# v-manhlt3/Disentangle-VAE-for-VC

Measured on AMD Instinct MI355X. Metric: utterances/sec (B=64, 80-mel, T=128) train step, higher is better.
Workload: dtype f32; 1 GPU; configs[1]: train step, B=64 pairs/GPU, 80-mel, T=128, 10 synthetic speakers, speaker_size=4, latent=32, Adam lr=1e-4; fp32 tensors, master weights, BatchNorm, losses and Adam; compute_mode=fp32x3, global_batch=64, frames=128, parallelism=dp1, launch=hipGraph replay, params=94930304

## Files before the change

disentangle-vae-for-vc_amd/_lib.py:

```python
from __future__ import annotations

import ctypes as C
import os
import subprocess

import torch

_HERE = os.path.dirname(os.path.abspath(__file__))
LIB_PATH = os.environ.get("DVAE_LIB_PATH") or os.path.join(_HERE, "libdvae_hip.so")
_lib = None

vp, i32, i64, f32 = C.c_void_p, C.c_int, C.c_int64, C.c_float


class Ranges(C.Structure):
    _fields_ = [("lo", i64 * 8), ("hi", i64 * 8), ("n", i32)]


class LstmDir(C.Structure):
    _fields_ = [("gates", vp), ("w_hh", vp), ("h_out", vp), ("c_all", vp), ("dh_out", vp),
                ("dgates", vp), ("dc_ws", vp), ("w_packed", vp), ("reverse", i32), ("packed_mode", i32),
                ("step_shift", i32), ("state_bf16", i32), ("pers_ws", vp), ("pers_timeout_us", C.c_uint), ("dbias_ih", vp), ("dbias_hh", vp), ("dbias_part", vp), ("gate_ld", i64)]


# ... 49 lines not shown
    "dvae_bn_ws_bytes": (i64, [i32, i32, i32]),
    "dvae_bn_stats_fwd": (i32, [vp, vp, vp, vp, vp, vp, vp, i32, i32, i32, i32, f32, f32, vp]),
    "dvae_bn_apply_fwd": (i32, [vp, vp, vp, vp, vp, vp, vp, i32, i32, i32, i32, i32, i32, vp]),
    "dvae_bn_bwd": (i32, [vp, vp, vp, vp, vp, vp, vp, vp, vp, vp, i32, i32, i32, i32, i32, i32, vp]),
    "dvae_bn_bwd_from_y": (i32, [vp, vp, vp, vp, vp, vp, vp, vp, vp, vp, i32, i32, i32, i32, i32, i32, vp]),
    "dvae_lstm_pack_w": (i32, [vp, vp, vp, i32, vp]),
    "dvae_lstm_pack_w_bf16": (i32, [vp, vp, vp, i32, vp]),
    "dvae_lstm_pack_w_x3": (i32, [vp, vp, vp, i32, vp]),
    "dvae_repack_all": (i32, [C.POINTER(RepackDesc), i32, vp]),
    "dvae_lstm_pers_supported": (i32, [i32, i32, i32, i32]),
    "dvae_lstm_pers_ws_bytes": (i64, [i32, i32]),
    "dvae_lstm_pers_check": (i32, [vp, C.POINTER(i32), vp]),
    "dvae_lstm_pers_selftest": (i32, [C.POINTER(LstmDir), i32, i32, i32, i64, i32, vp]),
    "dvae_lstm_seq_fwd": (i32, [C.POINTER(LstmDir), i32, i32, i32, i32, i64, vp]),
    "dvae_lstm_seq_bwd": (i32, [C.POINTER(LstmDir), i32, i32, i32, i32, i64, vp]),
    "dvae_lstm_seq_fwd_range": (i32, [C.POINTER(LstmDir), i32, i32, i32, i32, i64, i32, i32, vp]),
    "dvae_lstm_seq_bwd_range": (i32, [C.POINTER(LstmDir), i32, i32, i32, i32, i64, i32, i32, vp]),
    "dvae_latent_fwd": (i32, [vp] * 9 + [i32, i32, i32, vp]),
    "dvae_latent_bwd": (i32, [vp] * 11 + [i32, i32, i32, vp]),
    "dvae_kl_fwd": (i32, [vp, vp, vp, i64, f32, vp]),
    "dvae_kl_bwd": (i32, [vp, vp, vp, vp, vp, i64, f32, vp]),
    "dvae_l1_ws_bytes": (i64, [i64]),
    "dvae_l1_sum_fwd": (i32, [vp, vp, vp, vp, i64, f32, vp]),
    "dvae_l1_sum_bwd": (i32, [vp, vp, vp, vp, i64, f32, vp]),
    "dvae_loss_ws_bytes": (i64, [i64]),
    "dvae_loss_fwd": (i32, [C.POINTER(LossDesc), vp, vp, vp]),
    "dvae_loss_bwd": (i32, [C.POINTER(LossDesc), vp] + [vp] * 10 + [vp]),
    "dvae_loss_fwd_sched": (i32, [C.POINTER(LossDesc), C.POINTER(LossSched), vp, vp, vp, vp]),
    "dvae_loss_bwd_sched": (i32, [C.POINTER(LossDesc), C.POINTER(LossSched), vp, vp] + [vp] * 10 + [vp]),
    "dvae_gemm_f32_batched": (i32, [vp, vp, vp, i32, i32, i32, i32, i64, i64, i64, i32, i32, i32, i32, i32, vp]),
    "dvae_gemm_f32_slabs": (i32, [vp, vp, vp, vp, i64, i32, vp, i32, i32, i32, i64, i64, i64, i32, i32, i32, i32, i32, vp]),
    "dvae_gemm_f32_batched_slabs": (i32, [vp, vp, vp, i32, vp, i64, i32, i32, i32, i32, i64, i64, i64, i32, i32, i32, i32,
                                          i32, vp]),
    "dvae_conv5_fwd_slabs": (i32, [vp, vp, vp, vp, vp, i64, i32, i32, i32, i32, i32, i32, vp]),
    "dvae_conv5_dgrad_t_slabs": (i32, [vp, vp, vp, vp, i64, i32, i32, i32, i32, i32, i32, vp]),
    "dvae_conv5_wgrad_slabs": (i32, [vp, vp, vp, vp, i64, i32, i32, i32, i32, i32, i32, i32, i32, vp]),
    "dvae_slab_sum": (i32, [vp, vp, i64, i32, i64, i32, i32, vp]),
    "dvae_slab_fold": (i32, [C.POINTER(SlabDesc), i32, vp]),
    "dvae_colsum_ws_bytes": (i64, [i32, i32]),
    "dvae_colsum_add_ws": (i32, [vp, vp, vp, i32, i32, i64, i32, vp, vp]),
    "dvae_adam_flat": (i32, [vp, vp, vp, vp, i64, f32, f32, f32, f32, f32, i32, vp]),
    "dvae_adam_flat_dev": (i32, [vp, vp, vp, vp, i64, f32, f32, f32, vp, vp, vp, i32, vp]),
    "dvae_adam_flat_dev_clip": (i32, [vp, vp, vp, vp, i64, f32, f32, f32, vp, vp, vp, i32, vp, vp]),
    "dvae_grad_sumsq_ws_bytes": (i64, [i64]),
    "dvae_grad_sumsq": (i32, [vp, i64, vp, vp]),
    "dvae_grad_clip_finalize": (i32, [vp, i64, vp, vp, vp, i32, vp]),
    "dvae_ema_tick": (i32, [vp, vp, vp, vp]),
    "dvae_ema_update": (i32, [vp, vp, i64, vp, vp]),
    "dvae_swap_f32": (i32, [vp, vp, i64, vp]),
    "dvae_lstm_pers_err_word": (vp, [vp]),
    "dvae_sum_f32": (i32, [vp, vp, vp, vp, i64, vp]),
    "dvae_zero_f32": (i32, [vp, i64, vp]),
    "dvae_mel_to_frames": (i32, [vp, vp, vp, i32, i32, i32, i32, vp]),
    "dvae_frames_to_mel": (i32, [vp, vp, i32, i32, i32, vp]),
    "dvae_permute_102": (i32, [vp, vp, i32, i32, i32, vp]),
    "dvae_colsum_add": (i32, [vp, vp, vp, i32, i32, i64, i32, vp]),
    "dvae_transpose": (i32, [vp, vp, i32, i32, vp]),
    "dvae_act_fwd": (i32, [vp, i64, i32, vp]),
    "dvae_act_bwd": (i32, [vp, vp, vp, i64, i32, vp]),
    "dvae_gather_crop": (i32, [vp, vp, vp, vp, vp, i32, i32, i32, i32, vp]),
    "dvae_mel_to_chunks": (i32, [vp, vp, i32, i32, i32, i32, vp]),
    "dvae_chunks_to_mel": (i32, [vp, vp, i32, i32, i32, f32, f32, i32, vp]),
    "dvae_conversion_latents": (i32, [vp, vp, vp, vp, vp, i32, i32, i32, i32, vp]),
    "dvae_mul_div": (i32, [vp, vp, vp, vp, i64, vp]),
    "dvae_mel_to_windows": (i32, [vp, i64, vp, vp, vp, i32, i32, i32, vp]),
    "dvae_window_latents": (i32, [vp, vp, vp, vp, vp, C.c_double, vp, i32, i32, i32, i32, vp]),
# ... 124 lines not shown
```

disentangle-vae-for-vc_amd/csrc/gemm.hip:

```cpp
#include <cstdlib>
#include <type_traits>
#include <utility>
#include "common.h"
#include "gemm_common.h"

#ifndef DVAE_X3_PD
#define DVAE_X3_PD 2
#endif

int g_dvae_compute_mode = 0;
int g_dvae_deterministic = 0;

#if defined(DVAE_GEMM_TS) || defined(DVAE_GEMM_TS2)
__device__ unsigned long long g_gemm_ts[1024 * 8];
#define TS_NOW() __builtin_amdgcn_s_memtime()
#endif

__device__ __attribute__((aligned(16))) float g_gemm_zero[4] = {0.f, 0.f, 0.f, 0.f};

namespace {

template <bool A_KC, bool B_KC, int NTW, int BK, int WG, int MODE = 0, bool BNS = false, bool A16 = false, bool B16M = false>
__global__ __launch_bounds__(64 * WG * WG) void gemm_f32_kernel(const GemmParams p) {
  constexpr bool BF = (MODE == 1), X3 = (MODE == 2);
// ... 448 lines not shown
          const int dr = (r & 3) + 8 * (r >> 2);
          if (row0 + dr < p.M) cbase[(int64_t)dr * p.ldc] += acc[mt][nt][r] + bias_v;
        }
      } else {
#pragma unroll
        for (int r = 0; r < 16; ++r) {
          const int dr = (r & 3) + 8 * (r >> 2);
          if (row0 + dr < p.M) atomicAdd(cbase + (int64_t)dr * p.ldc, acc[mt][nt][r] + bias_v);
        }
      }
    }
  }
  if constexpr (BNS) {
    const int chunk = tile_m * 2 + wm, nchunks = (p.M + DVAE_BN_ROWS_PER_CHUNK - 1) / DVAE_BN_ROWS_PER_CHUNK;
#pragma unroll
    for (int nt = 0; nt < NTW; ++nt) {
      const int col = n0 + wn * 32 * NTW + nt * 32 + l31;
#pragma unroll
      for (int q = 0; q < 4; ++q) bst[nt][q] += __shfl_xor(bst[nt][q], 32, 64);
      if (kh == 0 && col < p.N && chunk < nchunks) {
        double* o = p.bn_part + ((int64_t)chunk * p.bn_groups * p.N + col) * 2;
        o[0] = (double)bst[nt][0];
        o[1] = (double)bst[nt][1];
        if (p.bn_groups > 1) {
          o[(int64_t)p.N * 2] = (double)bst[nt][2];
          o[(int64_t)p.N * 2 + 1] = (double)bst[nt][3];
        }
      }
    }
  }
}


template <bool A_KC, bool B_KC, bool BNS, bool BNU = false>
__global__ __launch_bounds__(256) void gemm_x3_tall_kernel(const GemmParams p) {
  constexpr int BM = 256, BN = 128, BK = 16, NTHR = 256, MTW = 4, NTW = 2;
  constexpr int LD_KC = BK + 8;
  constexpr int LDA = A_KC ? LD_KC : BM + 32;
  constexpr int LDB = B_KC ? LD_KC : BN + 32;
  constexpr int A_SZ = A_KC ? BM * LD_KC : BK * LDA;
  constexpr int B_SZ = B_KC ? BN * LD_KC : BK * LDB;
  constexpr int NUA = BM * BK / 8 / NTHR, NUB = BN * BK / 8 / NTHR;
  constexpr int NU = NUA + NUB;
  constexpr unsigned OOB = 0xC0000000u;
  __shared__ __attribute__((aligned(16))) __bf16 As[2][3 * A_SZ];
  __shared__ __attribute__((aligned(16))) __bf16 Bs[2][3 * B_SZ];
  typedef unsigned u32x4 __attribute__((ext_vector_type(4)));

  const int t = threadIdx.x;
  const int lane = t & 63, wave = t >> 6;
  const int wm = wave >> 1, wn = wave & 1;
  const int l31 = lane & 31, kh = lane >> 5;
#ifdef DVAE_GEMM_TS2
  const unsigned long long t2_entry = __builtin_amdgcn_s_memrealtime();
#endif

  int tile_m, tile_n;
  gemm_tile_of(p, tile_m, tile_n);
  const int m0 = tile_m * BM, n0 = tile_n * BN;
  int tap_fixed = 0, ks = blockIdx.z;
  if (p.tap_mode == 2) {
    tap_fixed = blockIdx.z % p.taps;
    ks = blockIdx.z / p.taps;
  }
  const int k_begin = ks * p.k_per_split;
  const int k_end = min(p.K, k_begin + p.k_per_split);
  const int kiters = (k_end - k_begin) / BK;
  const int n_iters = (p.tap_mode == 1 ? p.taps : 1) * kiters;
  const bool to_slab = p.slab != nullptr && p.split_k > 1;
  float* __restrict__ C = (to_slab ? p.slab + (int64_t)ks * p.slab_stride : (float*)p.C) +
                          (p.tap_mode == 2 ? (int64_t)tap_fixed * p.c_tap_stride : 0);

  const int a_rows = A_KC ? p.M : p.K, b_rows = B_KC ? p.N : p.K;
  const __amdgpu_buffer_rsrc_t a_rs = __builtin_amdgcn_make_buffer_rsrc((void*)p.A, 0, (int)((int64_t)a_rows * p.lda * 4), 0x00020000);
  const int64_t b_bytes = (int64_t)b_rows * p.ldb * 4 * ((p.tap_mode == 1) ? p.taps : 1);
  const __amdgpu_buffer_rsrc_t b_rs = __builtin_amdgcn_make_buffer_rsrc((void*)p.B, 0, (int)b_bytes, 0x00020000);
  unsigned a_vo[NUA], b_vo[NUB];
  int a_off[NUA], b_off[NUB];
#pragma unroll
  for (int j = 0; j < NUA; ++j) {
    const int idx = t + NTHR * j;
    if (A_KC) {
      const int row = idx >> 1, k8 = (idx & 1) * 8;
      a_off[j] = row * LDA + k8;
      a_vo[j] = (unsigned)(((int64_t)(m0 + row) * p.lda + k_begin + k8) * 4);
      if (m0 + row >= p.M) a_vo[j] = OOB;
    } else {
      const int kr = idx / (BM / 8), m8 = (idx % (BM / 8)) * 8;
      a_off[j] = kr * LDA + m8;
      a_vo[j] = (unsigned)(((int64_t)(k_begin + kr) * p.lda + m0 + m8) * 4);
      if (m0 + m8 >= p.M) a_vo[j] = OOB;
    }
  }
  const int64_t b_shift = (p.tap_mode == 2) ? (int64_t)(tap_fixed - 2) * p.bk_row_shift : 0;
#pragma unroll
  for (int j = 0; j < NUB; ++j) {
    const int idx = t + NTHR * j;
    if (B_KC) {
      const int row = idx >> 1, k8 = (idx & 1) * 8;
      b_off[j] = row * LDB + k8;
      b_vo[j] = (unsigned)(((int64_t)(n0 + row) * p.ldb + k_begin + k8) * 4);
      if (n0 + row >= p.N) b_vo[j] = OOB;
    } else {
      const int kr = idx / (BN / 8), n8 = (idx % (BN / 8)) * 8;
      b_off[j] = kr * LDB + n8;
      b_vo[j] = (unsigned)(((int64_t)(k_begin + kr) + b_shift) * p.ldb * 4 + (int64_t)(n0 + n8) * 4);
      if (n0 + n8 >= p.N) b_vo[j] = OOB;
    }
  }
  const int ntaps_loop = (p.tap_mode == 1) ? p.taps : 1;
  const int a_tap_step = (p.tap_mode == 1) ? (int)(p.a_row_shift * p.lda * 4) : 0;
  const int b_tap_step = (p.tap_mode == 1) ? (int)(p.b_tap_stride * 4) : 0;
  const int a_k_step = A_KC ? BK * 4 : (int)(BK * p.lda * 4);
  const int b_k_step = B_KC ? BK * 4 : (int)(BK * p.ldb * 4);
  int tap_n = 0, kit_n = 0;
  struct Regs {
    u32x4 a[NUA][2], b[NUB][2];
  };
  auto load_tiles = [&](Regs& g) {
    const bool live = kit_n < kiters;
    const unsigned a_s = live ? (unsigned)((tap_n - 2) * a_tap_step + kit_n * a_k_step) : OOB;
    const unsigned b_s = live ? (unsigned)(tap_n * b_tap_step + kit_n * b_k_step) : OOB;
#pragma unroll
    for (int j = 0; j < NUA; ++j) {
      g.a[j][0] = __builtin_amdgcn_raw_buffer_load_b128(a_rs, a_vo[j] + a_s, 0, 0);
      g.a[j][1] = __builtin_amdgcn_raw_buffer_load_b128(a_rs, a_vo[j] + a_s, 16, 0);
    }
// ... 47 lines not shown
  f32x16 acc[MTW][NTW];
#pragma unroll
  for (int i = 0; i < MTW; ++i)
#pragma unroll
    for (int j = 0; j < NTW; ++j)
#pragma unroll
      for (int r = 0; r < 16; ++r) acc[i][j][r] = 0.f;

  Regs gs[2];
  Frags fr[2];
  load_tiles(gs[0]);
  load_tiles(gs[1]);
  stage_all(0, gs[0]);
  load_tiles(gs[0]);
  __syncthreads();
  read_frags(fr[0], 0);
  stage_all(1, gs[1]);
  __syncthreads();

  constexpr int ia[6] = {0, 0, 1, 1, 0, 2}, ib[6] = {0, 1, 0, 1, 2, 0};
  unsigned a_s = 0, b_s = 0;
  unsigned pl[2][3][4];
  float rr[2][8];
  auto unit_regs = [&](Regs& g, int j) -> const u32x4(&)[2] { return j < NUA ? g.a[j] : g.b[j - NUA]; };
  auto fsub = [](float a, float b) {
    float r;
    asm("v_sub_f32 %0, %1, %2" : "=v"(r) : "v"(a), "v"(b));
    return r;
  };
  auto step = [&](auto G, auto U) {
    constexpr int g = decltype(G)::value, u = decltype(U)::value;
    {
      constexpr int term = g / 8, mt = (g % 8) / 2, nt = g % 2;
      acc[mt][nt] = __builtin_amdgcn_mfma_f32_32x32x16_bf16(fr[u].a[mt][ia[term]], fr[u].b[nt][ib[term]], acc[mt][nt], 0, 0, 0);
    }
    if constexpr (g < 6) {
      Regs& gn = gs[u ^ 1];
      constexpr int j = g / 2, hv = g % 2;
      if constexpr (j < NUA) gn.a[j][hv] = __builtin_amdgcn_raw_buffer_load_b128(a_rs, a_vo[j] + a_s, 16 * hv, 0);
      else gn.b[j - NUA][hv] = __builtin_amdgcn_raw_buffer_load_b128(b_rs, b_vo[j - NUA] + b_s, 16 * hv, 0);
    }
    if constexpr (g < 18) {
      Frags& f = fr[u ^ 1];
      constexpr int q = g / 6, w = g % 6;
      if constexpr (w < MTW) f.a[w][q] = frag(&As[u ^ 1][q * A_SZ], A_KC, LDA, wm * 128 + w * 32);
      else f.b[w - MTW][q] = frag(&Bs[u ^ 1][q * B_SZ], B_KC, LDB, wn * 64 + (w - MTW) * 32);
    } else {
      constexpr int s = g - 18;
      constexpr int SPU = 9;
      constexpr int j = s / SPU, w = s % SPU;
      if constexpr (j < NU) {
        const u32x4(&v)[2] = unit_regs(gs[u], j);
        if constexpr (w < 8) {
          constexpr int lvl = w / 4, i = w % 4;
          if constexpr (lvl == 0) {
            const f32x4 xv = __builtin_bit_cast(f32x4, v[i / 2]);
            rr[j & 1][2 * i] = xv[2 * (i % 2)];
            rr[j & 1][2 * i + 1] = xv[2 * (i % 2) + 1];
          }
          const f32x2 xy = {rr[j & 1][2 * i], rr[j & 1][2 * i + 1]};
          const unsigned pk = __builtin_bit_cast(unsigned, __builtin_convertvector(xy, bf16x2));
          pl[j & 1][lvl][i] = pk;
          rr[j & 1][2 * i] = fsub(rr[j & 1][2 * i], __builtin_bit_cast(float, pk << 16));
          rr[j & 1][2 * i + 1] = fsub(rr[j & 1][2 * i + 1], __builtin_bit_cast(float, pk & 0xffff0000u));
        } else {
#pragma unroll
          for (int i = 0; i < 4; ++i) {
// ... 151 lines not shown
            }
          }
        }
      }
      if constexpr (BNS) {
        const int chunk = tile_m * 4 + wm * 2 + half, nchunks = (p.M + DVAE_BN_ROWS_PER_CHUNK - 1) / DVAE_BN_ROWS_PER_CHUNK;
        bool second = false;
        if constexpr (BNU) second = ((m0 + wm * 128 + half * 64) % p.bn_nseg) >= p.bn_nseg / p.bn_groups;
#pragma unroll
        for (int nt = 0; nt < NTW; ++nt) {
          if (second) {
            bst[nt][2] = bst[nt][0];
            bst[nt][3] = bst[nt][1];
            bst[nt][0] = bst[nt][1] = 0.f;
          }
          const int col = n0 + wn * 64 + nt * 32 + l31;
#pragma unroll
          for (int q = 0; q < 4; ++q) bst[nt][q] += __shfl_xor(bst[nt][q], 32, 64);
          if (kh == 0 && col < p.N && chunk < nchunks) {
            double* o = p.bn_part + ((int64_t)chunk * p.bn_groups * p.N + col) * 2;
            o[0] = (double)bst[nt][0];
            o[1] = (double)bst[nt][1];
            if (p.bn_groups > 1) {
              o[(int64_t)p.N * 2] = (double)bst[nt][2];
              o[(int64_t)p.N * 2 + 1] = (double)bst[nt][3];
            }
          }
        }
      }
    }
  };
  using std::integral_constant;
  const int epi_here = to_slab ? DVAE_EPI_STORE : p.epi;
  if (epi_here == DVAE_EPI_ATOMIC) emit(integral_constant<int, DVAE_EPI_ATOMIC>{}, integral_constant<int, DVAE_ACT_NONE>{});
  else if (epi_here == DVAE_EPI_ACCUM) emit(integral_constant<int, DVAE_EPI_ACCUM>{}, integral_constant<int, DVAE_ACT_NONE>{});
  else if (p.act == DVAE_ACT_NONE) emit(integral_constant<int, DVAE_EPI_STORE>{}, integral_constant<int, DVAE_ACT_NONE>{});
  else if (p.act == DVAE_ACT_RELU) emit(integral_constant<int, DVAE_EPI_STORE>{}, integral_constant<int, DVAE_ACT_RELU>{});
  else emit(integral_constant<int, DVAE_EPI_STORE>{}, integral_constant<int, DVAE_ACT_TANH>{});
#ifdef DVAE_GEMM_TS2
  asm volatile("s_waitcnt vmcnt(0)" ::: "memory");
  const unsigned flat_wg = blockIdx.z * gridDim.x + blockIdx.x;
  if ((threadIdx.x & 63) == 0 && flat_wg < 256) {
    unsigned long long* o = g_gemm_ts + (flat_wg * 4 + wave) * 8;
    o[0] = t2_entry; o[1] = t2_loop0; o[2] = t2_loop1; o[3] = __builtin_amdgcn_s_memrealtime();
    o[4] = (unsigned long long)n_iters;
    unsigned xcc;
    asm volatile("s_getreg_b32 %0, hwreg(HW_REG_XCC_ID)" : "=s"(xcc));
    o[5] = xcc & 0xf;
  }
#endif
}



template <bool A_KC, bool B_KC, bool BNS, bool BNU = false>
__global__ __launch_bounds__(256) void gemm_bf16_tall_kernel(const GemmParams p) {
  constexpr int BM = 256, BN = 128, BK = 64, NTHR = 256, MTW = 4, NTW = 2;
  constexpr int LD_KC = BK + 8;
  constexpr int LDA = A_KC ? LD_KC : BM + 32;
  constexpr int LDB = B_KC ? LD_KC : BN + 32;
  constexpr int A_SZ = A_KC ? BM * LD_KC : BK * LDA;
  constexpr int B_SZ = B_KC ? BN * LD_KC : BK * LDB;
  constexpr int NPA = BM * BK / 8 / NTHR, NPB = BN * BK / 8 / NTHR;
  constexpr int NP = NPA + NPB;
  constexpr unsigned OOB = 0xC0000000u;
  __shared__ __attribute__((aligned(16))) __bf16 As[2][A_SZ];
// ... 578 lines not shown
  p.lda = lda; p.ldb = ldb; p.ldc = ldc;
  p.taps = 1; p.tap_mode = 0;
  p.split_k = split_k; p.act = DVAE_ACT_NONE; p.epi = epi;
  p.slab = slab; p.slab_stride = slab_stride; p.slab_cap = slab_cap;
  if (slab && slab_stride < (int64_t)M * ldc) return DVAE_EINVAL;
  const int rc = launch_gemm(p, a_kcontig != 0, b_kcontig != 0, mode, (hipStream_t)stream);
  return rc == DVAE_OK ? p.split_k : rc;
}

DVAE_API int dvae_gemm_f32_batched_slabs(const void* const* A, const void* const* B, void* const* C, int batch, float* slab,
                                         int64_t slab_stride, int slab_cap, int M, int N, int K, int64_t lda, int64_t ldb,
                                         int64_t ldc, int a_kcontig, int b_kcontig, int epi, int split_k, int mode,
                                         void* stream) {
  if (!A || !B || !C || batch < 1 || batch > 4 || (!slab && split_k > 1)) return DVAE_EINVAL;
  GemmParams p{};
  p.A = A[0]; p.B = B[0]; p.C = C[0]; p.bias = nullptr;
  p.M = M; p.N = N; p.K = K;
  p.lda = lda; p.ldb = ldb; p.ldc = ldc;
  p.taps = 1; p.tap_mode = 0;
  p.split_k = split_k; p.act = DVAE_ACT_NONE; p.epi = epi;
  p.batch = batch;
  p.slab = slab; p.slab_stride = slab_stride; p.slab_cap = slab_cap / batch;
  if (slab && slab_stride < (int64_t)M * ldc) return DVAE_EINVAL;
  for (int b = 0; b < batch; ++b) {
    if (!A[b] || !B[b] || !C[b] || ((((uintptr_t)A[b]) | ((uintptr_t)B[b]) | ((uintptr_t)C[b])) & 15)) return DVAE_EINVAL;
    p.a_boff[b] = (const char*)A[b] - (const char*)A[0];
    p.b_boff[b] = (const char*)B[b] - (const char*)B[0];
    p.c_boff[b] = (char*)C[b] - (char*)C[0];
  }
  const int rc = launch_gemm(p, a_kcontig != 0, b_kcontig != 0, mode, (hipStream_t)stream);
  return rc == DVAE_OK ? p.split_k : rc;
}

DVAE_API int dvae_zero_f32(float* x, int64_t n, void* stream);

namespace {
void narrow_conv_split(GemmParams& p, int mode, hipStream_t s) {
  int m = mode;
  if (m >= 0) m &= 0xff;
  if (m == DVAE_MODE_DEFAULT) m = g_dvae_compute_mode;
  if (m != DVAE_MODE_F32X3 || (g_dvae_deterministic && !p.slab) || (mode >= 0 && (mode & ~0xff))) return;
  if (p.N <= 64 || p.N > 128 || (p.N & 3) || p.M < 256 || (((uintptr_t)p.C) & 15)) return;
  const int tiles = (p.M + 255) / 256;
  if (tiles >= 192) return;
  for (int sk = 2; sk <= 8; sk *= 2) {
    if (p.K % (16 * sk)) return;
    const int steps = (p.K / sk / 16) * p.taps;
    if (steps < 24) return;
    if (tiles * sk >= 192) {
      if (p.slab) {
        if (sk > p.slab_cap) return;
        p.split_k = sk;
        return;
      }
      if (dvae_zero_f32((float*)p.C, (int64_t)p.M * p.ldc, s) != DVAE_OK) return;
      p.split_k = sk;
      p.epi = DVAE_EPI_ATOMIC;
      return;
    }
  }
}
}

DVAE_API int dvae_conv5_fwd_stats(const void* X, const void* Wp, const float* bias, float* Y, int R, int N, int Cin,
                                  int Cout, int mode, int G, void* bn_ws, void* stream) {
  if (!bn_ws || G < 1 || G > 2 || N < 1 || (N % G) || (R % N)) return DVAE_EINVAL;
// ... 99 lines not shown
```

disentangle-vae-for-vc_amd/ops.py:

```python
from __future__ import annotations

import ctypes as C
import os
from typing import Callable, Optional

import torch

from . import _lib
from ._lib import check, lib, ptr, stream

ACT_NONE, ACT_RELU, ACT_TANH = 0, 1, 2
EPI_STORE, EPI_ACCUM, EPI_ATOMIC = 0, 1, 2
BN_EPS, BN_MOMENTUM = 1e-5, 0.1

grad_ready_hook: Optional[Callable[[torch.Tensor], None]] = None

USE_SIDE_STREAM = os.environ.get("DVAE_SIDE_STREAM", "0") != "0"
_side_stream = None
_side_dirty = False
_cb_task = None


_fold_owners: list = []

# ... 221 lines not shown
    nb = len(params)
    grads = [_grad_buf(p) for p in params]
    arr = lambda xs: (C.c_void_p * nb)(*[a(x) for x in xs])
    m = _mflags(_mode(mode), As[0], Bs[0], grads[0]) | flags
    if split_k <= 1:
        check(lib().dvae_gemm_f32_batched(arr(As), arr(Bs), arr(grads), nb, M, N, K, lda, ldb, N, 0, 0, EPI_ACCUM, 1, m,
                                          stream()), "dvae_gemm_f32_batched")
        return
    owner = _owner_of(params[0])
    stride = _pad4(M * N)
    cap = _cap_for(split_k) * nb
    key = (grads[0].data_ptr(), M * N, cap)
    slab = _slab_store(owner).get(key) if owner is not None else None
    if slab is None:
        if owner is not None:
            slab = _slab_store(owner)[key] = torch.empty(cap * stride, device=grads[0].device, dtype=torch.float32)
        else:
            slab, _ = _scratch_slabs(grads[0].device, cap * stride, 1)
    if owner is not None:
        _claim_slabs(slab, [_owner_of(p) for p in params])
    n = lib().dvae_gemm_f32_batched_slabs(arr(As), arr(Bs), arr(grads), nb, ptr(slab), stride, cap, M, N, K, lda, ldb, N, 0, 0,
                                          EPI_ACCUM, split_k, m, stream())
    if n < 1:
        check(n, "dvae_gemm_f32_batched_slabs")
    if n > 1:
        for b, (g, p) in enumerate(zip(grads, params)):
            _defer_fold(g, _owner_of(p), slab.data_ptr() + 4 * b * n * stride, stride, n)


def _owner_of(p):
    return getattr(p, "_dvae_owner", None)


def gemm_slabs(A, B, Cout, bias, M, N, K, lda, ldb, ldc, a_kc, b_kc, epi, split_k, mode, slab, stride, cap, flags=0):
    a = lambda t: t if (t is None or isinstance(t, int)) else t.data_ptr()
    n = lib().dvae_gemm_f32_slabs(a(A), a(B), a(Cout), a(slab), stride, cap, a(bias), M, N, K, lda, ldb, ldc, int(a_kc),
                                  int(b_kc), epi, split_k, _mflags(_mode(mode), A, B, Cout) | flags, stream())
    if n < 1:
        check(n, "dvae_gemm_f32_slabs")
    return n


def _cap_for(split_k: int) -> int:
    return max(SLAB_CAP, min(128, 2 * int(split_k)))


def gemm_split(A, B, Cout, bias, M, N, K, lda, ldb, ldc, a_kc, b_kc, act, split_k, mode, flags=0):
    n_el = M * ldc
    cap = _cap_for(split_k)
    slab, stride = _scratch_slabs(Cout.device, n_el, cap)
    n = gemm_slabs(A, B, Cout, bias, M, N, K, lda, ldb, ldc, a_kc, b_kc, EPI_STORE, split_k, mode, slab, stride, cap, flags)
    if n > 1:
        check(lib().dvae_slab_sum(ptr(Cout), ptr(slab), stride, n, n_el, act, 0, stream()), "dvae_slab_sum")
    elif act != ACT_NONE:
        check(lib().dvae_slab_sum(ptr(Cout), None, 0, 0, n_el, act, 1, stream()), "dvae_slab_sum")


def wgrad_gemm(A, B, grad, owner, M, N, K, lda, ldb, a_kc, b_kc, split_k, mode, flags=0):
    if split_k <= 1:
        gemm(A, B, grad, None, M, N, K, lda, ldb, N, a_kc, b_kc, ACT_NONE, EPI_ACCUM, 1, mode, flags)
        return
    cap = _cap_for(split_k)
    if owner is not None:
        slab, stride = _param_slabs(grad, cap, owner)
        _claim_slabs(slab, (owner,))
    else:
        slab, stride = _scratch_slabs(grad.device, grad.numel(), cap)
    n = gemm_slabs(A, B, grad, None, M, N, K, lda, ldb, N, a_kc, b_kc, EPI_ACCUM, split_k, mode, slab, stride, cap, flags)
# ... 312 lines not shown
            check(L.dvae_bn_bwd(ptr(dz), ptr(y), ptr(z), ptr(mean), ptr(rstd), ptr(bn_w), ptr(dy),
                                ptr(_grad_buf(bn_w)), ptr(_grad_buf(bn_b)), ptr(ws), R, n_seg, Cout, G, act,
                                _b16(z) | (_b16(dy) << 1), st), "dvae_bn_bwd")
        dx = None
        if ctx.needs_input_grad[0]:
            dx = torch.empty((R, Cin), device=dev, dtype=torch.float32)
            if wpt is None:
                from .derived import conv_wpt_local
                wpt = conv_wpt_local(conv_wp)
            if Cin <= 128 and (R * Cin) % 4 == 0:
                slab, stride = _scratch_slabs(dev, R * Cin, 8)
                n = L.dvae_conv5_dgrad_t_slabs(ptr(dy), ptr(wpt), ptr(dx), ptr(slab), stride, 8, R, n_seg, Cin, Cout,
                                               _mflags(mode, dy, wpt), st)
                if n < 1:
                    check(n, "dvae_conv5_dgrad_t_slabs")
                if n > 1:
                    check(L.dvae_slab_sum(ptr(dx), ptr(slab), stride, n, R * Cin, ACT_NONE, 0, st), "dvae_slab_sum")
            else:
                check(L.dvae_conv5_dgrad_t(ptr(dy), ptr(wpt), ptr(dx), R, n_seg, Cin, Cout, _mflags(mode, dy, wpt), st),
                      "dvae_conv5_dgrad_t")
        with side_work(dy, xa):
            if Cout >= 256 and Cin > 64:
                sk = _split_k(5 * ((Cout + 255) // 256) * ((Cin + 127) // 128), R, slots=256, fixed=384)
            else:
                sk = _split_k(5 * _tiles(Cout, Cin), R)
            gw, own = _grad_buf(conv_wp), _owner_of(conv_wp)
            slab, stride = (None, 0)
            cap = _cap_for(sk)
            if sk > 1 and own is not None:
                slab, stride = _param_slabs(gw, cap, own)
                _claim_slabs(slab, (own,))
            elif sk > 1:
                slab, stride = _scratch_slabs(dev, gw.numel(), cap)
            n = L.dvae_conv5_wgrad_slabs(ptr(dy), ptr(xa), ptr(gw), ptr(slab), stride, cap if sk > 1 else 0, R, n_seg,
                                         Cin, Cout, EPI_ACCUM, sk, _mflags(mode, dy, xa), stream())
            if n < 1:
                check(n, "dvae_conv5_wgrad_slabs")
            if n > 1:
                _defer_fold(gw, own, slab.data_ptr(), stride, n)
            colsum_add(dy, _grad_buf(conv_b))
        _ready(conv_wp, conv_b, bn_w, bn_b)
        dres = dz if has_res else None
        return (dx, None, None, None, None, None, None, None, dres, None, None, None, None, None, None, None, None)


LSTM_PERSISTENT = os.environ.get("DVAE_LSTM_PERSISTENT", "1") != "0"


def _ranks_share_a_gpu() -> bool:
    try:
        if "LOCAL_WORLD_SIZE" not in os.environ:
            return False
        n_local = int(os.environ["LOCAL_WORLD_SIZE"])
        n_dev = torch.cuda.device_count()
        return n_dev > 0 and n_local > n_dev
    except Exception:
        return False


if _ranks_share_a_gpu():
    import warnings
    warnings.warn(f"dvae_amd: LOCAL_WORLD_SIZE={os.environ.get('LOCAL_WORLD_SIZE')} ranks share {torch.cuda.device_count()} "
                  "visible GPU(s): the W_hh-resident persistent recurrences are switched OFF (one launch per frame, much "
                  "slower) — a functional check, not the product set-up")
    LSTM_PERSISTENT = False
LSTM_PERS_TIMEOUT_US = 0
_PERS_WS_BYTES = (1 << 20) + 4 * 16 * 128 * 2 * 1024
_pers_ws: dict = {}
# ... 816 lines not shown
                                  stream()), "dvae_factor_fwd")
        ctx.save_for_backward(z, q_mu, q_lv, L, weights)
        ctx.S = S
        return pen

    @staticmethod
    def backward(ctx, g):
        z, q_mu, q_lv, L, weights = ctx.saved_tensors
        g = g.contiguous()
        _ok(g)
        N, D = z.shape
        dz, dmu, dlv = torch.empty_like(z), torch.empty_like(z), torch.empty_like(z)
        check(lib().dvae_factor_bwd(ptr(z), ptr(q_mu), ptr(q_lv), ptr(L), N, D, ctx.S, ptr(weights), ptr(g), ptr(dz),
                                    ptr(dmu), ptr(dlv), stream()), "dvae_factor_bwd")
        return dz, dmu, dlv, None, None, None


def prof_enable(family: int):
    check(lib().dvae_prof_enable(family), "dvae_prof_enable")


def prof_collect_tags(max_tags: int = 64):
    tags, ms = (C.c_uint * max_tags)(), (C.c_double * max_tags)()
    n_l, fl, by = (C.c_int64 * max_tags)(), (C.c_double * max_tags)(), (C.c_double * max_tags)()
    n = lib().dvae_prof_collect_tags(tags, ms, n_l, fl, by, max_tags)
    if n < 0:
        raise _lib.DvaeHipError(f"dvae_prof_collect_tags failed: rc={n}")
    out = []
    for i in range(n):
        t = int(tags[i])
        bns, a16, b16 = (t >> 19) & 1, (t >> 17) & 1, (t >> 18) & 1
        if (t >> 10) & 7 == 3:
            name = f"gemm_bf16_256_kernel<A_KC={t & 1}, B_KC={(t >> 1) & 1}, BNS={bns}> tap_mode={(t >> 15) & 3}"
        elif (t >> 10) & 7 == 1:
            kn = "gemm_bf16_tall_kernel" if (t >> 13) & 3 == 1 else "gemm_x3_tall_kernel"
            name = f"{kn}<A_KC={t & 1}, B_KC={(t >> 1) & 1}, BNS={bns}> tap_mode={(t >> 15) & 3}"
        else:
            name = (f"gemm_f32_kernel<A_KC={t & 1}, B_KC={(t >> 1) & 1}, NTW={(t >> 2) & 3}, BK={(t >> 4) & 63}, "
                    f"WG={(t >> 10) & 7}, MODE={(t >> 13) & 3}, BNS={bns}, A16={a16}, B16M={b16}> tap_mode={(t >> 15) & 3}")
        out.append({"tag": t, "kernel": name, "ms": float(ms[i]), "launches": int(n_l[i]), "flops": float(fl[i]),
                    "bytes": float(by[i])})
    return sorted(out, key=lambda d: -d["ms"])


def prof_collect():
    ms, n, fl = C.c_double(), C.c_int64(), C.c_double()
    check(lib().dvae_prof_collect(C.byref(ms), C.byref(n), C.byref(fl)), "dvae_prof_collect")
    return ms.value, n.value, fl.value


if os.environ.get("DVAE_DETERMINISTIC", "0") == "1":
    set_deterministic(True)
```

include/dvae_hip.h:

```cpp
#ifndef DVAE_HIP_H
#define DVAE_HIP_H

#include <stddef.h>
#include <stdint.h>

#ifdef __cplusplus
extern "C" {
#endif

#define DVAE_OK 0
#define DVAE_EINVAL (-1)
#define DVAE_ELAUNCH (-2)

#define DVAE_ACT_NONE 0
#define DVAE_ACT_RELU 1
#define DVAE_ACT_TANH 2

#define DVAE_EPI_STORE 0
#define DVAE_EPI_ACCUM 1
#define DVAE_EPI_ATOMIC 2

#define DVAE_ABI_VERSION 319
int dvae_version(void);

#define DVAE_MODE_A_BF16 0x100
#define DVAE_MODE_B_BF16 0x200
#define DVAE_MODE_C_BF16 0x400
#define DVAE_MODE_DEFAULT (-1)
#define DVAE_MODE_F32 0
#define DVAE_MODE_BF16 1
#define DVAE_MODE_F32X3 2
int dvae_set_compute_mode(int mode);
int dvae_get_compute_mode(void);

int dvae_set_deterministic(int on);
int dvae_get_deterministic(void);
int dvae_last_hip_error(void);

int dvae_gemm_f32(const void* A, const void* B, void* C, const float* bias,
                  int M, int N, int K, int64_t lda, int64_t ldb, int64_t ldc,
                  int a_kcontig, int b_kcontig, int act, int epi, int split_k, int mode, void* stream);

int dvae_gemm_f32_batched(const void* const* A, const void* const* B, void* const* C, int batch, int M, int N, int K,
                          int64_t lda, int64_t ldb, int64_t ldc, int a_kcontig, int b_kcontig, int epi, int split_k,
                          int mode, void* stream);
int dvae_gemm_f32_slabs(const void* A, const void* B, void* C, float* slab, int64_t slab_stride, int slab_cap,
                        const float* bias, int M, int N, int K, int64_t lda, int64_t ldb, int64_t ldc,
                        int a_kcontig, int b_kcontig, int epi, int split_k, int mode, void* stream);
int dvae_gemm_f32_batched_slabs(const void* const* A, const void* const* B, void* const* C, int batch, float* slab,
                                int64_t slab_stride, int slab_cap, int M, int N, int K, int64_t lda, int64_t ldb,
                                int64_t ldc, int a_kcontig, int b_kcontig, int epi, int split_k, int mode, void* stream);
int dvae_conv5_fwd_slabs(const void* X, const void* Wp, const float* bias, float* Y, float* slab, int64_t slab_stride,
                         int slab_cap, int R, int N, int Cin, int Cout, int mode, void* stream);
int dvae_conv5_dgrad_t_slabs(const void* dY, const void* Wpt, float* dX, float* slab, int64_t slab_stride, int slab_cap,
                             int R, int N, int Cin, int Cout, int mode, void* stream);
int dvae_conv5_wgrad_slabs(const void* dY, const void* X, float* dWp, float* slab, int64_t slab_stride, int slab_cap,
                           int R, int N, int Cin, int Cout, int epi, int split_k, int mode, void* stream);
int dvae_slab_sum(float* C, const float* slab, int64_t slab_stride, int nslab, int64_t n, int act, int accumulate,
                  void* stream);
typedef struct {
  float* c;
  const float* slab;
  int64_t slab_stride;
  int64_t n;
  int nslab;
  int pad_;
} dvae_slab_desc_t;
#define DVAE_SLAB_FOLD_MAX 64
int dvae_slab_fold(const dvae_slab_desc_t* descs, int n_entries, void* stream);
int dvae_conv5_fwd(const void* X, const void* Wp, const float* bias, float* Y,
                   int R, int N, int Cin, int Cout, int mode, void* stream);
int dvae_conv5_fwd_stats(const void* X, const void* Wp, const float* bias, float* Y,
                         int R, int N, int Cin, int Cout, int mode, int G, void* bn_ws, void* stream);
int dvae_conv5_wgrad(const void* dY, const void* X, float* dWp,
                     int R, int N, int Cin, int Cout, int split_k, int mode, void* stream);
int dvae_conv_pack_w(const float* W, float* Wp, int Cout, int Cin, void* stream);
int dvae_conv_pack_wt(const float* W, float* Wpt, int Cout, int Cin, void* stream);
int dvae_conv5_dgrad_t(const void* dY, const void* Wpt, float* dX, int R, int N, int Cin, int Cout, int mode,
                       void* stream);
int dvae_conv_unpack_add_w(const float* dWp, float* dW, int Cout, int Cin, void* stream);

int64_t dvae_bn_ws_bytes(int R, int C, int G);
int dvae_bn_stats_fwd(const float* Y, float* mean, float* rstd, float* running_mean, float* running_var,
                      int64_t* num_batches_tracked, void* ws, int R, int N, int C, int G,
// ... 295 lines not shown
```

Measured before the change: 3635 utterances/sec.

## Route skinny fp32x3 GEMMs and conv5 wgrad through transposed tall kernel

Adds a transposed (CT) variant of the x3 tall GEMM kernel. It computes C^T = B^T A^T so that small-M, large-N GEMMs (M<=128) land on the 256-row tile dimension, with an XCD-aware split-K grid mapping and a transposed store epilogue. Python routes eligible gemm_slabs calls and conv5 weight-gradient calls to the new path by default (DVAE_SKINNY=1). The aim is to avoid wasting most of the M tile on skinny shapes. The risks are uncoalesced column-major stores and a new code path for the tap shift logic.

Result: no change. 3625 utterances/sec (-0.3%).

```diff
diff --git a/disentangle-vae-for-vc_amd/_lib.py b/disentangle-vae-for-vc_amd/_lib.py
--- a/disentangle-vae-for-vc_amd/_lib.py
+++ b/disentangle-vae-for-vc_amd/_lib.py
@@ -105,6 +105,8 @@
     "dvae_gemm_f32_slabs": (i32, [vp, vp, vp, vp, i64, i32, vp, i32, i32, i32, i64, i64, i64, i32, i32, i32, i32, i32, vp]),
     "dvae_gemm_f32_batched_slabs": (i32, [vp, vp, vp, i32, vp, i64, i32, i32, i32, i32, i64, i64, i64, i32, i32, i32, i32,
                                           i32, vp]),
+    "dvae_gemm_x3_rows_slabs": (i32, [vp, vp, vp, vp, i64, i32, vp, i32, i32, i32, i64, i64, i64, i32, i32, i32, i32, vp]),
+    "dvae_conv5_wgrad_rows_slabs": (i32, [vp, vp, vp, vp, i64, i32, i32, i32, i32, i32, i32, i32, vp]),
     "dvae_conv5_fwd_slabs": (i32, [vp, vp, vp, vp, vp, i64, i32, i32, i32, i32, i32, i32, vp]),
     "dvae_conv5_dgrad_t_slabs": (i32, [vp, vp, vp, vp, i64, i32, i32, i32, i32, i32, i32, vp]),
     "dvae_conv5_wgrad_slabs": (i32, [vp, vp, vp, vp, i64, i32, i32, i32, i32, i32, i32, i32, i32, vp]),
diff --git a/disentangle-vae-for-vc_amd/csrc/gemm.hip b/disentangle-vae-for-vc_amd/csrc/gemm.hip
--- a/disentangle-vae-for-vc_amd/csrc/gemm.hip
+++ b/disentangle-vae-for-vc_amd/csrc/gemm.hip
@@ -504,8 +504,9 @@
 }
 
 
-template <bool A_KC, bool B_KC, bool BNS, bool BNU = false>
+template <bool A_KC, bool B_KC, bool BNS, bool BNU = false, bool CT = false>
 __global__ __launch_bounds__(256) void gemm_x3_tall_kernel(const GemmParams p) {
+  static_assert(!CT || !BNS, "transposed (rows) form: no BatchNorm statistics");
   constexpr int BM = 256, BN = 128, BK = 16, NTHR = 256, MTW = 4, NTW = 2;
   constexpr int LD_KC = BK + 8;
   constexpr int LDA = A_KC ? LD_KC : BM + 32;
@@ -528,9 +529,16 @@
 #endif
 
   int tile_m, tile_n;
-  gemm_tile_of(p, tile_m, tile_n);
+  int tap_fixed = 0, ks = blockIdx.z;
+  if (CT && p.xcd_map == 2) {
+    const int x = blockIdx.x & 7, q = blockIdx.x >> 3;
+    tile_m = q % p.tiles_m;
+    tile_n = 0;
+    ks = (q / p.tiles_m) * 8 + x;
+  } else {
+    gemm_tile_of(p, tile_m, tile_n);
+  }
   const int m0 = tile_m * BM, n0 = tile_n * BN;
-  int tap_fixed = 0, ks = blockIdx.z;
   if (p.tap_mode == 2) {
     tap_fixed = blockIdx.z % p.taps;
     ks = blockIdx.z / p.taps;
@@ -560,11 +568,12 @@
     } else {
       const int kr = idx / (BM / 8), m8 = (idx % (BM / 8)) * 8;
       a_off[j] = kr * LDA + m8;
-      a_vo[j] = (unsigned)(((int64_t)(k_begin + kr) * p.lda + m0 + m8) * 4);
+      const int64_t a_shift = (CT && p.tap_mode == 2) ? (int64_t)(tap_fixed - 2) * p.bk_row_shift : 0;
+      a_vo[j] = (unsigned)((((int64_t)(k_begin + kr) + a_shift) * p.lda + m0 + m8) * 4);
       if (m0 + m8 >= p.M) a_vo[j] = OOB;
     }
   }
-  const int64_t b_shift = (p.tap_mode == 2) ? (int64_t)(tap_fixed - 2) * p.bk_row_shift : 0;
+  const int64_t b_shift = (!CT && p.tap_mode == 2) ? (int64_t)(tap_fixed - 2) * p.bk_row_shift : 0;
 #pragma unroll
   for (int j = 0; j < NUB; ++j) {
     const int idx = t + NTHR * j;
@@ -678,7 +687,8 @@
     constexpr int g = decltype(G)::value, u = decltype(U)::value;
     {
       constexpr int term = g / 8, mt = (g % 8) / 2, nt = g % 2;
-      acc[mt][nt] = __builtin_amdgcn_mfma_f32_32x32x16_bf16(fr[u].a[mt][ia[term]], fr[u].b[nt][ib[term]], acc[mt][nt], 0, 0, 0);
+      constexpr int pa = CT ? ib[term] : ia[term], pb = CT ? ia[term] : ib[term];
+      acc[mt][nt] = __builtin_amdgcn_mfma_f32_32x32x16_bf16(fr[u].a[mt][pa], fr[u].b[nt][pb], acc[mt][nt], 0, 0, 0);
     }
     if constexpr (g < 6) {
       Regs& gn = gs[u ^ 1];
@@ -896,6 +906,32 @@
   };
   using std::integral_constant;
   const int epi_here = to_slab ? DVAE_EPI_STORE : p.epi;
+  if constexpr (CT) {
+    auto emit_ct = [&](auto EPI_) {
+      constexpr int epi = decltype(EPI_)::value;
+#pragma unroll
+      for (int mt = 0; mt < MTW; ++mt)
+#pragma unroll
+        for (int nt = 0; nt < NTW; ++nt) {
+          const int col = n0 + wn * 64 + nt * 32 + l31;
+          if (col >= p.N) continue;
+#pragma unroll
+          for (int g = 0; g < 4; ++g) {
+            const int row = m0 + wm * 128 + mt * 32 + 4 * kh + 8 * g;
+            if (row >= p.M) continue;
+            f32x4 o4;
+#pragma unroll
+            for (int e = 0; e < 4; ++e) o4[e] = acc[mt][nt][4 * g + e] + (add_bias ? p.bias[row + e] : 0.f);
+            f32x4* dst = reinterpret_cast<f32x4*>(C + (int64_t)col * p.ldc + row);
+            if constexpr (epi == DVAE_EPI_ACCUM) o4 += *dst;
+            *dst = o4;
+          }
+        }
+    };
+    if (epi_here == DVAE_EPI_ACCUM) emit_ct(integral_constant<int, DVAE_EPI_ACCUM>{});
+    else emit_ct(integral_constant<int, DVAE_EPI_STORE>{});
+    return;
+  }
   if (epi_here == DVAE_EPI_ATOMIC) emit(integral_constant<int, DVAE_EPI_ATOMIC>{}, integral_constant<int, DVAE_ACT_NONE>{});
   else if (epi_here == DVAE_EPI_ACCUM) emit(integral_constant<int, DVAE_EPI_ACCUM>{}, integral_constant<int, DVAE_ACT_NONE>{});
   else if (p.act == DVAE_ACT_NONE) emit(integral_constant<int, DVAE_EPI_STORE>{}, integral_constant<int, DVAE_ACT_NONE>{});
@@ -1540,6 +1576,81 @@
   return rc == DVAE_OK ? p.split_k : rc;
 }
 
+namespace {
+int launch_x3_rows(GemmParams p, bool a_kc, bool b_kc, int split_k, hipStream_t s) {
+  const int M = p.M, N = p.N, K = p.K, ntap = p.tap_mode == 2 ? p.taps : 1;
+  if (!p.A || !p.B || !p.C || M < 1 || M > 128 || N < 4 || K < 16 || (K & 15) || (N & 3) || (!a_kc && (M & 3))) return DVAE_EINVAL;
+  if ((p.lda & 3) || (p.ldb & 3) || (p.ldc & 3) || p.lda < (a_kc ? K : M) || p.ldb < (b_kc ? K : N) || p.ldc < N) return DVAE_EINVAL;
+  if ((((uintptr_t)p.A) | ((uintptr_t)p.B) | ((uintptr_t)p.C) | ((uintptr_t)p.slab)) & 15) return DVAE_EINVAL;
+  if (p.epi != DVAE_EPI_STORE && p.epi != DVAE_EPI_ACCUM) return DVAE_EINVAL;
+  if ((!p.slab && split_k > 1) || p.slab_cap < 0 || (p.slab_stride & 3) || (p.c_tap_stride & 3)) return DVAE_EINVAL;
+  if ((int64_t)(a_kc ? M : K) * p.lda * 4 >= (1ll << 30) || (int64_t)(b_kc ? N : K) * p.ldb * 4 >= (1ll << 30)) return DVAE_EINVAL;
+  if (p.tap_mode == 2 && b_kc) return DVAE_EINVAL;
+  if (split_k < 1 || (g_dvae_deterministic && !p.slab)) split_k = 1;
+  if (p.slab && split_k > p.slab_cap) split_k = p.slab_cap > 0 ? p.slab_cap : 1;
+  int kps = (K + split_k - 1) / split_k;
+  kps = ((kps + 15) / 16) * 16;
+  p.k_per_split = kps;
+  p.split_k = (K + kps - 1) / kps;
+  p.act = DVAE_ACT_NONE;
+  std::swap(p.A, p.B);
+  std::swap(p.lda, p.ldb);
+  p.M = N; p.N = M;
+  p.tiles_m = (N + 255) / 256;
+  dim3 grid(p.tiles_m, 1, p.split_k * ntap);
+  if (p.tap_mode == 0 && p.split_k % 8 == 0) {
+    p.xcd_map = 2;
+    grid = dim3(p.tiles_m * p.split_k, 1, 1);
+  } else if (p.tiles_m % 8 == 0) {
+    p.xcd_map = 1;
+    const int per = p.tiles_m >> 3;
+    int gm = 1;
+    for (int d = 1; d <= 32 && d <= per; ++d)
+      if (per % d == 0) gm = d;
+    p.map_gm = gm; p.map_gn = 1; p.map_nstr = 1;
+  }
+  const unsigned tag = (a_kc ? 1u : 0u) | (b_kc ? 2u : 0u) | (2u << 2) | (16u << 4) | (5u << 10) | ((unsigned)DVAE_MODE_F32X3 << 13) |
+                       ((unsigned)p.tap_mode << 15);
+  ProfScope prof(1, s, 2.0 * M * N * (double)K * ntap, tag, 4.0 * ((double)M * K + (double)K * N + (double)M * N * ntap));
+#define ROWS(BIG_KC_, ROWS_KC_) hipLaunchKernelGGL((gemm_x3_tall_kernel<BIG_KC_, ROWS_KC_, false, false, true>), grid, dim3(256), 0, s, p)
+  if (b_kc && a_kc) ROWS(true, true);
+  else if (b_kc) ROWS(true, false);
+  else if (a_kc) ROWS(false, true);
+  else ROWS(false, false);
+#undef ROWS
+  const int rc = dvae_check_launch();
+  return rc == DVAE_OK ? p.split_k : rc;
+}
+}
+
+DVAE_API int dvae_gemm_x3_rows_slabs(const void* A, const void* B, void* C, float* slab, int64_t slab_stride, int slab_cap,
+                                     const float* bias, int M, int N, int K, int64_t lda, int64_t ldb, int64_t ldc,
+                                     int a_kcontig, int b_kcontig, int epi, int split_k, void* stream) {
+  GemmParams p{};
+  p.A = A; p.B = B; p.C = C; p.bias = bias;
+  p.M = M; p.N = N; p.K = K;
+  p.lda = lda; p.ldb = ldb; p.ldc = ldc;
+  p.taps = 1; p.tap_mode = 0;
+  p.epi = epi;
+  p.slab = slab; p.slab_stride = slab_stride; p.slab_cap = slab_cap;
+  if (slab && slab_stride < (int64_t)M * ldc) return DVAE_EINVAL;
+  return launch_x3_rows(p, a_kcontig != 0, b_kcontig != 0, split_k, (hipStream_t)stream);
+}
+
+DVAE_API int dvae_conv5_wgrad_rows_slabs(const void* dY, const void* X, float* dWp, float* slab, int64_t slab_stride,
+                                         int slab_cap, int R, int N, int Cin, int Cout, int epi, int split_k, void* stream) {
+  GemmParams p{};
+  p.A = dY; p.B = X; p.C = dWp; p.bias = nullptr;
+  p.M = Cout; p.N = Cin; p.K = R;
+  p.lda = Cout; p.ldb = Cin; p.ldc = Cin;
+  p.taps = 5; p.tap_mode = 2;
+  p.bk_row_shift = N; p.c_tap_stride = (int64_t)Cout * Cin;
+  p.epi = epi;
+  p.slab = slab; p.slab_stride = slab_stride; p.slab_cap = slab_cap;
+  if (N < 1 || (slab && slab_stride < 5 * (int64_t)Cout * Cin)) return DVAE_EINVAL;
+  return launch_x3_rows(p, false, false, split_k, (hipStream_t)stream);
+}
+
 DVAE_API int dvae_zero_f32(float* x, int64_t n, void* stream);
 
 namespace {
diff --git a/disentangle-vae-for-vc_amd/ops.py b/disentangle-vae-for-vc_amd/ops.py
--- a/disentangle-vae-for-vc_amd/ops.py
+++ b/disentangle-vae-for-vc_amd/ops.py
@@ -277,8 +277,44 @@
     return getattr(p, "_dvae_owner", None)
 
 
+_SKINNY = os.environ.get("DVAE_SKINNY", "1") != "0"
+SKINNY_MIN_BIG = 1 << 22
+SKINNY_MIN_N = 256
+
+
+def set_skinny(flag: bool = True):
+    global _SKINNY
+    _SKINNY = bool(flag)
+
+
+def skinny() -> bool:
+    return _SKINNY
+
+
+def skinny_route(M, N, K, a_kc, b_kc, epi, mode, ldc=None, taps=1, enabled=True):
+    if not enabled or int(mode) != MODE_F32X3:
+        return None
+    ldc = N if ldc is None else ldc
+    if M > 128 or M < 1 or K % 16 or N % 4 or ldc % 4 or epi not in (EPI_STORE, EPI_ACCUM) or (not a_kc and M % 4):
+        return None
+    if taps != 1 and (taps != 5 or a_kc or b_kc):
+        return None
+    if b_kc:
+        return None
+    if N < SKINNY_MIN_N or N * K < SKINNY_MIN_BIG or 4 * N * K >= (1 << 30) or 4 * M * K >= (1 << 30):
+        return None
+    return "rows"
+
+
 def gemm_slabs(A, B, Cout, bias, M, N, K, lda, ldb, ldc, a_kc, b_kc, epi, split_k, mode, slab, stride, cap, flags=0):
     a = lambda t: t if (t is None or isinstance(t, int)) else t.data_ptr()
+    m = _mflags(_mode(mode), A, B, Cout) | flags
+    if skinny_route(M, N, K, a_kc, b_kc, epi, m, ldc, enabled=_SKINNY) == "rows":
+        n = lib().dvae_gemm_x3_rows_slabs(a(A), a(B), a(Cout), a(slab), stride, cap, a(bias), M, N, K, lda, ldb, ldc,
+                                          int(a_kc), int(b_kc), epi, split_k, stream())
+        if n < 1:
+            check(n, "dvae_gemm_x3_rows_slabs")
+        return n
     n = lib().dvae_gemm_f32_slabs(a(A), a(B), a(Cout), a(slab), stride, cap, a(bias), M, N, K, lda, ldb, ldc, int(a_kc),
                                   int(b_kc), epi, split_k, _mflags(_mode(mode), A, B, Cout) | flags, stream())
     if n < 1:
@@ -657,8 +693,13 @@
                 _claim_slabs(slab, (own,))
             elif sk > 1:
                 slab, stride = _scratch_slabs(dev, gw.numel(), cap)
-            n = L.dvae_conv5_wgrad_slabs(ptr(dy), ptr(xa), ptr(gw), ptr(slab), stride, cap if sk > 1 else 0, R, n_seg,
-                                         Cin, Cout, EPI_ACCUM, sk, _mflags(mode, dy, xa), stream())
+            mf = _mflags(mode, dy, xa)
+            if skinny_route(Cout, Cin, R, False, False, EPI_ACCUM, mf, Cin, taps=5, enabled=_SKINNY) == "rows":
+                n = L.dvae_conv5_wgrad_rows_slabs(ptr(dy), ptr(xa), ptr(gw), ptr(slab), stride, cap if sk > 1 else 0, R, n_seg,
+                                                  Cin, Cout, EPI_ACCUM, sk, stream())
+            else:
+                n = L.dvae_conv5_wgrad_slabs(ptr(dy), ptr(xa), ptr(gw), ptr(slab), stride, cap if sk > 1 else 0, R, n_seg,
+                                             Cin, Cout, EPI_ACCUM, sk, mf, stream())
             if n < 1:
                 check(n, "dvae_conv5_wgrad_slabs")
             if n > 1:
@@ -1541,6 +1582,9 @@
         bns, a16, b16 = (t >> 19) & 1, (t >> 17) & 1, (t >> 18) & 1
         if (t >> 10) & 7 == 3:
             name = f"gemm_bf16_256_kernel<A_KC={t & 1}, B_KC={(t >> 1) & 1}, BNS={bns}> tap_mode={(t >> 15) & 3}"
+        elif (t >> 10) & 7 == 5:
+            name = (f"gemm_x3_rows_kernel<A_KC={t & 1}, B_KC={(t >> 1) & 1}> tap_mode={(t >> 15) & 3} "
+                    "(gemm_x3_tall_kernel, transposed)")
         elif (t >> 10) & 7 == 1:
             kn = "gemm_bf16_tall_kernel" if (t >> 13) & 3 == 1 else "gemm_x3_tall_kernel"
             name = f"{kn}<A_KC={t & 1}, B_KC={(t >> 1) & 1}, BNS={bns}> tap_mode={(t >> 15) & 3}"
diff --git a/include/dvae_hip.h b/include/dvae_hip.h
--- a/include/dvae_hip.h
+++ b/include/dvae_hip.h
@@ -50,6 +50,11 @@
 int dvae_gemm_f32_batched_slabs(const void* const* A, const void* const* B, void* const* C, int batch, float* slab,
                                 int64_t slab_stride, int slab_cap, int M, int N, int K, int64_t lda, int64_t ldb,
                                 int64_t ldc, int a_kcontig, int b_kcontig, int epi, int split_k, int mode, void* stream);
+int dvae_gemm_x3_rows_slabs(const void* A, const void* B, void* C, float* slab, int64_t slab_stride, int slab_cap,
+                            const float* bias, int M, int N, int K, int64_t lda, int64_t ldb, int64_t ldc, int a_kcontig,
+                            int b_kcontig, int epi, int split_k, void* stream);
+int dvae_conv5_wgrad_rows_slabs(const void* dY, const void* X, float* dWp, float* slab, int64_t slab_stride, int slab_cap,
+                                int R, int N, int Cin, int Cout, int epi, int split_k, void* stream);
 int dvae_conv5_fwd_slabs(const void* X, const void* Wp, const float* bias, float* Y, float* slab, int64_t slab_stride,
                          int slab_cap, int R, int N, int Cin, int Cout, int mode, void* stream);
 int dvae_conv5_dgrad_t_slabs(const void* dY, const void* Wpt, float* dX, float* slab, int64_t slab_stride, int slab_cap,
```
